# ApricityXX/PaddlePaddle

Measured on AMD Instinct MI355X. Metric: tokens/sec GPT-3-13B sharding-3 + ResNet50 img/s, at 1/2/4/8 MI355X, higher is better.
Workload: dtype bf16; 1 GPU; model=GPT-3 13B (h5120 L40 a40 ffn20480 V50304), global_batch=16, seq_len=2048, micro_batch=4, accum_steps=4, parallelism=sharding_stage3_degree1, recompute=False, fused_head_ce=False, paired_wgrad=False, optimizer=AdamW fp32-master fused HIP, amp=O2 bf16, allocator=native auto-growth best-fit

## Files before the change

### csrc/kernels/flash_attn_kernels.h

```cpp
#pragma once
#include "common.h"
#include "mfma_tile.h"

using namespace pa;

typedef __attribute__((ext_vector_type(8))) _Float16 f16x8_t;
typedef __attribute__((ext_vector_type(16))) float f32x16;

namespace pa_fa {

constexpr float kLog2e = 1.4426950408889634f;
constexpr float kLn2 = 0.6931471805599453f;

union Frag {
  bf16x8_t v;
  f16x8_t f;
  uint4 u;
  s16x4 h[2];
};

template <bool F16>
__device__ __forceinline__ f32x16 mfma32(const Frag& a, const Frag& b, f32x16 c) {
  if constexpr (F16) return __builtin_amdgcn_mfma_f32_32x32x16_f16(a.f, b.f, c, 0, 0, 0);
  else return __builtin_amdgcn_mfma_f32_32x32x16_bf16(a.v, b.v, c, 0, 0, 0);
// ... 606 lines not shown
  const int h0 = hk * G;
  const int64_t dq_row0 = varlen ? (int64_t)q_start : (int64_t)b * p.Sq;
  auto head_range = [&](int h, int& qa, int& qe) {
    qa = q_begin0;
    qe = Sq;
    if constexpr (kFm) {
      if (p.fm_stats != nullptr) {
        const int* st = p.fm_stats + (int64_t)b * p.fmst[0] + (int64_t)h * p.fmst[1] + (int64_t)(kb * (BK / 64)) * 8;
        int mx_lo0 = st[1], mn_lo1 = st[2], mx_up0 = st[5], mn_up1 = st[6];
#pragma unroll
        for (int tt = 1; tt < BK / 64; ++tt) {
          mx_lo0 = max(mx_lo0, st[tt * 8 + 1]); mn_lo1 = min(mn_lo1, st[tt * 8 + 2]);
          mx_up0 = max(mx_up0, st[tt * 8 + 5]); mn_up1 = min(mn_up1, st[tt * 8 + 6]);
        }
        if (mn_lo1 == 0x7fffffff) qe = min(qe, max(mx_lo0, 0));
        if (mx_up0 <= 0) qa = max(qa, min(mn_up1, Sq));
      }
    }
    qa = (qa / BM) * BM;
  };

  constexpr int QLOADS = BM * NCH / NT;
  u32x4 qreg[QLOADS], dreg[QLOADS];
  constexpr int mk = kMk;
  constexpr bool has_fm = kFm;
  float lse_raw = 0.f, dlt_raw = 0.f;
  uint32_t mreg[16];
  bool row_ok = false;
  bool q_ok[QLOADS];
  auto prefetch = [&](int h, int q0) {
    const uint16_t* qbase = p.q + (varlen ? (int64_t)q_start * p.qs[1] : (int64_t)b * p.qs[0]) + (int64_t)h * p.qs[2];
    const uint16_t* dobase =
        p.dout + (varlen ? (int64_t)q_start * p.dos[1] : (int64_t)b * p.dos[0]) + (int64_t)h * p.dos[2];
#pragma unroll
    for (int i = 0; i < QLOADS; ++i) {
      const int idx = tid + NT * i;
      const int row = idx / NCH, ch = idx % NCH;
      const int qx = q0 + row;
      q_ok[i] = qx < Sq;
      const int qc = q_ok[i] ? qx : Sq - 1;
      qreg[i] = gload16_async(qbase + (int64_t)qc * p.qs[1] + ch * 8);
      dreg[i] = gload16_async(dobase + (int64_t)qc * p.dos[1] + ch * 8);
    }
    const int qx = q0 + (tid & (BM - 1));
    row_ok = qx < Sq;
    const int qc = row_ok ? qx : Sq - 1;
    const int64_t lrow = (int64_t)b * p.lse_s[0] + (int64_t)h * p.lse_s[1] + q_start + qc;
    lse_raw = __uint_as_float(gload4_async(p.lse + lrow));
    dlt_raw = __uint_as_float(gload4_async(p.delta + lrow));
  };
  auto mask_load = [&](int h, int q0) {
    if constexpr (kMask) {
      constexpr int esz = kMk == kMaskBool ? 1 : (kMk == kMaskBF16 ? 2 : 4);
      const char* mb = reinterpret_cast<const char*>(p.mask) + ((int64_t)b * p.ms[0] + (int64_t)h * p.ms[1]) * esz;
      const int kc = kj < Sk ? kj : 0;
#pragma unroll
      for (int i = 0; i < 16; ++i) {
        int qr = q0 + (i & 3) + 8 * (i >> 2) + 4 * hf;
        qr = qr < Sq ? qr : 0;
        const char* ad = mb + ((int64_t)qr * p.ms[2] + kc) * esz;
        if constexpr (kMk == kMaskBool) mreg[i] = gload1_async(ad);
        else if constexpr (kMk == kMaskBF16) mreg[i] = gload2_async(ad);
        else mreg[i] = gload4_async(ad);
      }
    }
  };
  const bool has_atomics = w < NDT;
  const float inv_scale = 1.f / p.scale;

  auto dq_step = [&](const char* dsb, int h, int qb0) {
    float* dqb = p.dq_acc + dq_row0 * p.H * D + (int64_t)h * D;
    const __amdgpu_buffer_rsrc_t dq_rsrc = __builtin_amdgcn_make_buffer_rsrc(
        dqb, 0, (int)((int64_t)(Sq - 1) * p.H * D * 4 + D * 4), 0x00020000);
    for (int dt = w; dt < NDT; dt += NW) {
      f32x16 qacc = zero16();
#pragma unroll
      for (int ks = 0; ks < BK / 16; ++ks) {
        Frag a, bb;
        const int kr0 = 16 * ks + 8 * hf;
        const int ra = kr0 + qq, rb = kr0 + 4 + qq;
        a.h[0] = lds_tr(dsb + (ra * (BM * 2) + (((16 * G1 + 4 * pp) * 2) ^ (((ra >> 2) & 3) << 3))));
        a.h[1] = lds_tr(dsb + (rb * (BM * 2) + (((16 * G1 + 4 * pp) * 2) ^ (((rb >> 2) & 3) << 3))));
        const int cch = (dt * 32 + 16 * G1) / 8 + (pp >> 1);
        bb.h[0] = lds_tr(k_lds + (img_off<NCH>(kr0 + qq, cch) + 8 * (pp & 1)));
        bb.h[1] = lds_tr(k_lds + (img_off<NCH>(kr0 + 4 + qq, cch) + 8 * (pp & 1)));
        qacc = mfma32<F16>(a, bb, qacc);
      }
      const int rs = p.H * D * 4;
      const int base = qb0 * rs + (dt * 32 + r) * 4;
#pragma unroll
      for (int i = 0; i < 16; ++i) {
        const int qr = (i & 3) + 8 * (i >> 2) + 4 * hf;
        const int off = (qb0 + qr < Sq && !(p.abl & 1)) ? base + qr * rs : 0x7ffffff0;
        __builtin_amdgcn_raw_ptr_buffer_atomic_fadd_f32(qacc[i] * p.scale, dq_rsrc, off, 0, 0);
      }
    }
  };


  for (int hi = 0; hi < G; ++hi) {
    const int h = h0 + hi;
    int qa, qe;
    head_range(h, qa, qe);
    const int n_qb = qa < qe ? (qe - qa + BM - 1) / BM : 0;
    if (n_qb == 0) continue;
    FmBounds fbk{0, 0, 0, 0};
    if constexpr (kFm) {
      const int* fbp = p.fm + (int64_t)b * p.fms[0] + (int64_t)h * p.fms[1] + (int64_t)(kj < Sk ? kj : 0) * p.fm_cols;
      int v4[4];
#pragma unroll
      for (int j = 0; j < 4; ++j) v4[j] = fbp[j < p.fm_cols ? j : 0];
      fbk = fm_canon(v4, p.fm_cols, p.causal);
    }
    prefetch(h, qa);
    for (int it = 0; it < n_qb; ++it) {
      const int q0 = qa + it * BM;
      if (it == 0 || !has_atomics || ATOMICS > 63) {
        asm volatile("s_waitcnt vmcnt(0)" : "+v"(qreg[0]), "+v"(dreg[0]), "+v"(lse_raw), "+v"(dlt_raw)::"memory");
      } else {
        asm volatile("s_waitcnt vmcnt(%4)" : "+v"(qreg[0]), "+v"(dreg[0]), "+v"(lse_raw), "+v"(dlt_raw)
                     : "n"(ATOMICS > 63 ? 0 : ATOMICS) : "memory");
      }
      if constexpr (QLOADS > 1) asm volatile("" : "+v"(qreg[QLOADS - 1]), "+v"(dreg[QLOADS - 1]));
#pragma unroll
      for (int i = 0; i < QLOADS; ++i) {
        if (!q_ok[i]) {
          qreg[i] = u32x4{0u, 0u, 0u, 0u};
          dreg[i] = u32x4{0u, 0u, 0u, 0u};
        }
      }
      const float lse_r = row_ok ? -lse_raw * inv_scale : -INFINITY;
      const float dlt_r = row_ok ? -dlt_raw : 0.f;
      lds_barrier();
#pragma unroll
      for (int i = 0; i < QLOADS; ++i) {
        const int idx = tid + NT * i;
        const int row = idx / NCH, ch = idx % NCH;
        *reinterpret_cast<u32x4*>(q_lds + img_off<NCH>(row, ch)) = qreg[i];
        *reinterpret_cast<u32x4*>(do_lds + img_off<NCH>(row, ch)) = dreg[i];
      }
      if (tid < BM) {
        lse_s[tid] = lse_r;
        dlt_s[tid] = dlt_r;
      }
      lds_barrier();
      if (kMask) mask_load(h, q0);
      if (it + 1 < n_qb) prefetch(h, q0 + BM);
      if (it > 0 && !(p.abl & 2)) dq_step(ds_lds + (((it - 1) & 1) * DST_BYTES), h, q0 - BM);
      const bool dq_ran = it > 0 && has_atomics;

      f32x16 sacc, pacc;
#pragma unroll
      for (int g = 0; g < 4; ++g) {
        const float4 l4 = *reinterpret_cast<const float4*>(lse_s + 8 * g + 4 * hf);
        const float4 d4 = *reinterpret_cast<const float4*>(dlt_s + 8 * g + 4 * hf);
        sacc[4 * g + 0] = l4.x; sacc[4 * g + 1] = l4.y; sacc[4 * g + 2] = l4.z; sacc[4 * g + 3] = l4.w;
        pacc[4 * g + 0] = d4.x; pacc[4 * g + 1] = d4.y; pacc[4 * g + 2] = d4.z; pacc[4 * g + 3] = d4.w;
      }
#pragma unroll
      for (int ks = 0; ks < KS; ++ks) {
        Frag qa, da;
        qa.u = lds_b128(q_lds, img_off<NCH>(r, 2 * ks + hf));
        da.u = lds_b128(do_lds, img_off<NCH>(r, 2 * ks + hf));
        if constexpr (CACHE_KV) {
          sacc = mfma32<F16>(qa, kfr[ks], sacc);
          pacc = mfma32<F16>(da, vfr[ks], pacc);
        } else {
          Frag kk, vv;
          kk.u = lds_b128(k_lds, img_off<NCH>(w * 32 + r, 2 * ks + hf));
          vv.u = lds_b128(v_lds, img_off<NCH>(w * 32 + r, 2 * ks + hf));
          sacc = mfma32<F16>(qa, kk, sacc);
          pacc = mfma32<F16>(da, vv, pacc);
        }
      }
      if constexpr (kMask) {
        const int n_after = (it + 1 < n_qb ? 2 * QLOADS + 2 : 0) + (dq_ran ? ATOMICS : 0);
        switch (n_after) {
          case 4: asm volatile("s_waitcnt vmcnt(4)" : "+v"(mreg[0]), "+v"(mreg[15]) :: "memory"); break;
          case 6: asm volatile("s_waitcnt vmcnt(6)" : "+v"(mreg[0]), "+v"(mreg[15]) :: "memory"); break;
          case 16: asm volatile("s_waitcnt vmcnt(16)" : "+v"(mreg[0]), "+v"(mreg[15]) :: "memory"); break;
          case 18: asm volatile("s_waitcnt vmcnt(18)" : "+v"(mreg[0]), "+v"(mreg[15]) :: "memory"); break;
          case 20: asm volatile("s_waitcnt vmcnt(20)" : "+v"(mreg[0]), "+v"(mreg[15]) :: "memory"); break;
          case 22: asm volatile("s_waitcnt vmcnt(22)" : "+v"(mreg[0]), "+v"(mreg[15]) :: "memory"); break;
          case 34: asm volatile("s_waitcnt vmcnt(34)" : "+v"(mreg[0]), "+v"(mreg[15]) :: "memory"); break;
          default: asm volatile("s_waitcnt vmcnt(0)" : "+v"(mreg[0]), "+v"(mreg[15]) :: "memory"); break;
        }
#pragma unroll
        for (int i = 1; i < 15; ++i) asm volatile("" : "+v"(mreg[i]));
      }
      if (kMask && (mk == kMaskBF16 || mk == kMaskF32)) {
#pragma unroll
        for (int i = 0; i < 16; ++i) {
          const float madd = mk == kMaskBF16 ? lo_bf16(mreg[i]) : __uint_as_float(mreg[i]);
          sacc[i] += madd * inv_scale;
        }
      }
      const bool need_mask = kj >= Sk || (p.causal && kb * BK + BK - 1 > q0 + shift) || mk == kMaskBool || kFm;
      const uint32_t ka = (uint32_t)(kj >> 1);
#pragma unroll
      for (int i = 0; i < 16; ++i) {
        const int qr = (i & 3) + 8 * (i >> 2) + 4 * hf;
        float pr = __builtin_amdgcn_exp2f(sacc[i] * p.scale_log2);
        if (need_mask) {
          bool dead = kj >= Sk || (p.causal && kj > q0 + qr + shift);
          if (kMask && mk == kMaskBool) dead = dead || (mreg[i] & 0xFFu) == 0u;
          if (kFm) dead = dead || fm_masked(fbk, q0 + qr);
          if (dead) pr = 0.f;
        }
        if (kDrop) {
          const uint32_t qa = (uint32_t)(q0 + qr) ^ ((uint32_t)(b * p.H + h) * 0x9E3779B1u);
          const bool keep = drop_keep(drop_hash(p.seed0, p.seed1, qa, ka), kj, p.keep16);
          const float ndelta = dlt_s[qr];
          const float dp = pacc[i] - ndelta;
          pacc[i] = pr * ((keep ? dp * p.rkeep : 0.f) + ndelta);
          sacc[i] = keep ? pr * p.rkeep : 0.f;
        } else {
          sacc[i] = pr;
          pacc[i] = pr * pacc[i];
        }
      }
      Frag pf[2], sf[2];
#pragma unroll
      for (int s = 0; s < 2; ++s) {
        float a[8], cc[8];
#pragma unroll
        for (int j = 0; j < 8; ++j) { a[j] = sacc[8 * s + j]; cc[j] = pacc[8 * s + j]; }
        pf[s] = pack8<F16>(a);
        sf[s] = pack8<F16>(cc);
      }

#pragma unroll
      for (int dt = 0; dt < NDT; ++dt) {
        if (p.abl & 4) break;
        const int cch = (dt * 32 + 16 * G1) / 8 + (pp >> 1);
        const int cb = 8 * (pp & 1);
#pragma unroll
        for (int s = 0; s < 2; ++s) {
          const int R0 = 16 * s + 4 * hf;
          Frag a, cfr;
          a.h[0] = lds_tr(do_lds + (img_off<NCH>(R0 + qq, cch) + cb));
          a.h[1] = lds_tr(do_lds + (img_off<NCH>(R0 + 8 + qq, cch) + cb));
          dv_acc[dt] = mfma32<F16>(a, pf[s], dv_acc[dt]);
          cfr.h[0] = lds_tr(q_lds + (img_off<NCH>(R0 + qq, cch) + cb));
          cfr.h[1] = lds_tr(q_lds + (img_off<NCH>(R0 + 8 + qq, cch) + cb));
          dk_acc[dt] = mfma32<F16>(cfr, sf[s], dk_acc[dt]);
        }
      }

      {
        const int row = w * 32 + r;
        char* rowp = ds_lds + (it & 1) * DST_BYTES + row * (BM * 2);
        const int sw = ((row >> 2) & 3) << 3;
#pragma unroll
        for (int s = 0; s < 2; ++s) {
          const Frag f = sf[s];
          *reinterpret_cast<uint2*>(rowp + (((16 * s + 4 * hf) * 2) ^ sw)) = make_uint2(f.u.x, f.u.y);
          *reinterpret_cast<uint2*>(rowp + (((16 * s + 8 + 4 * hf) * 2) ^ sw)) = make_uint2(f.u.z, f.u.w);
        }
      }
    }
    lds_barrier();
    if (!(p.abl & 2)) dq_step(ds_lds + (((n_qb - 1) & 1) * DST_BYTES), h, qa + (n_qb - 1) * BM);
  }

  if (kj < Sk) {
    uint16_t* dkrow = p.dk + (varlen ? (int64_t)k_start * p.dks[1] : (int64_t)b * p.dks[0]) + (int64_t)kj * p.dks[1] +
                      (int64_t)hk * p.dks[2];
    uint16_t* dvrow = p.dv + (varlen ? (int64_t)k_start * p.dvs[1] : (int64_t)b * p.dvs[0]) + (int64_t)kj * p.dvs[1] +
                      (int64_t)hk * p.dvs[2];
#pragma unroll
    for (int dt = 0; dt < NDT; ++dt) {
#pragma unroll
      for (int g = 0; g < 4; ++g) {
        const int d0 = dt * 32 + 8 * g + 4 * hf;
        uint2 a, cc;
        a.x = pack2<F16>(dk_acc[dt][4 * g] * p.scale, dk_acc[dt][4 * g + 1] * p.scale);
        a.y = pack2<F16>(dk_acc[dt][4 * g + 2] * p.scale, dk_acc[dt][4 * g + 3] * p.scale);
        cc.x = pack2<F16>(dv_acc[dt][4 * g], dv_acc[dt][4 * g + 1]);
        cc.y = pack2<F16>(dv_acc[dt][4 * g + 2], dv_acc[dt][4 * g + 3]);
        *reinterpret_cast<uint2*>(dkrow + d0) = a;
        *reinterpret_cast<uint2*>(dvrow + d0) = cc;
      }
    }
  }
}



template <bool F16>
__device__ __forceinline__ f32x4 mfma16(const Frag& a, const Frag& b, f32x4 c) {
  if constexpr (F16) return __builtin_amdgcn_mfma_f32_16x16x32_f16(a.f, b.f, c, 0, 0, 0);
  else return __builtin_amdgcn_mfma_f32_16x16x32_bf16(a.v, b.v, c, 0, 0, 0);
}

__device__ __forceinline__ int fa_swz(int row) { return (0x78 >> (2 * ((row >> 2) & 3))) & 3; }
__device__ __forceinline__ int img_a(int row, int ch) {
  return 2048 * (row >> 3) + 512 * (ch >> 2) + 64 * (row & 7) + 16 * ((ch & 3) ^ fa_swz(row));
}

__device__ __forceinline__ int dst_off(int row, int col4) {
  return row * 64 + ((col4 ^ ((row >> 1) & 7)) << 3);
}

template <bool F16, bool DSQ>
__global__ __launch_bounds__(512, 1) void fa_bwd16_kernel(BwdArgs p) {
  constexpr int D = 128, NCH = 16, NW = 8, NT = NW * 64, BK = 128, BM = 32;
  constexpr int KT_BYTES = BK * D * 2;
  constexpr int QT_BYTES = BM * D * 2;
  constexpr int DST_BYTES = BK * BM * 2;
  __shared__ __attribute__((aligned(16))) char smem[2 * KT_BYTES + 4 * QT_BYTES + 2 * DST_BYTES + 2 * 2 * BM * 4];
  char* k_lds = smem;
  char* v_lds = smem + KT_BYTES;
  char* q_st = v_lds + KT_BYTES;
  char* do_st = q_st + 2 * QT_BYTES;
  char* ds_lds = do_st + 2 * QT_BYTES;
  char* rc_st = ds_lds + 2 * DST_BYTES;

  const int nkb0 = (p.Sk + BK - 1) / BK;
  int kb, bhk;
  block_map((int)blockIdx.x, p.B * p.Hk, nkb0, p.grp, bhk, kb);
  const int b = bhk / p.Hk, hk = bhk % p.Hk;
  const int G = p.H / p.Hk;
  int q_start = 0, k_start = 0, Sq = p.Sq, Sk = p.Sk;
  const bool varlen = p.cu_q != nullptr;
  if (varlen) {
    q_start = p.cu_q[b];
    Sq = p.cu_q[b + 1] - q_start;
    k_start = p.cu_k[b];
    Sk = p.cu_k[b + 1] - k_start;
  }
  if (kb * BK >= Sk) return;
  const int tid = threadIdx.x, w = tid >> 6, lane = tid & 63, r16 = lane & 15, kg = lane >> 4;
  const int tq = r16 >> 2, tp = r16 & 3;
  const int shift = Sk - Sq;
  const int kj = kb * BK + w * 16 + r16;

  const uint16_t* kbase = p.k + (varlen ? (int64_t)k_start * p.ks[1] : (int64_t)b * p.ks[0]) + (int64_t)hk * p.ks[2];
  const uint16_t* vbase = p.v + (varlen ? (int64_t)k_start * p.vs[1] : (int64_t)b * p.vs[0]) + (int64_t)hk * p.vs[2];
#pragma unroll
  for (int i = 0; i < BK * NCH / NT; ++i) {
    const int idx = tid + NT * i;
    const int row = idx / NCH, ch = idx % NCH;
    const int key = kb * BK + row;
    uint4 val = make_uint4(0, 0, 0, 0), vv = make_uint4(0, 0, 0, 0);
    if (key < Sk) {
      val = *reinterpret_cast<const uint4*>(kbase + (int64_t)key * p.ks[1] + ch * 8);
      vv = *reinterpret_cast<const uint4*>(vbase + (int64_t)key * p.vs[1] + ch * 8);
    }
    *reinterpret_cast<uint4*>(k_lds + img_a(row, ch)) = val;
    *reinterpret_cast<uint4*>(v_lds + img_a(row, ch)) = vv;
  }
  f32x4 dk_acc[8], dv_acc[8];
#pragma unroll
  for (int dt = 0; dt < 8; ++dt)
#pragma unroll
    for (int i = 0; i < 4; ++i) { dk_acc[dt][i] = 0.f; dv_acc[dt][i] = 0.f; }
  __syncthreads();
  Frag kfr[4], vfr[4];
#pragma unroll
  for (int ks = 0; ks < 4; ++ks) {
    kfr[ks].u = lds_b128(k_lds, img_a(w * 16 + r16, 4 * ks + kg));
    vfr[ks].u = lds_b128(v_lds, img_a(w * 16 + r16, 4 * ks + kg));
  }

  int q_begin0 = 0;
  if (p.causal) q_begin0 = max(0, kb * BK - shift);
  q_begin0 = DSQ ? (q_begin0 / 128) * 128 : (q_begin0 / BM) * BM;
  const int h0 = hk * G;
  const int64_t dq_row0 = varlen ? (int64_t)q_start : (int64_t)b * p.Sq;

  const int o_dst = 1024 * w + 16 * lane;
  const int pf_row = 8 * (o_dst >> 11) + ((o_dst & 511) >> 6);
  const int pf_ch = 4 * ((o_dst & 2047) >> 9) + (((o_dst & 63) >> 4) ^ fa_swz(pf_row));
  auto prefetch = [&](int h, int q0, int sl) {
    const uint16_t* qbase = p.q + (varlen ? (int64_t)q_start * p.qs[1] : (int64_t)b * p.qs[0]) + (int64_t)h * p.qs[2];
    const uint16_t* dobase =
        p.dout + (varlen ? (int64_t)q_start * p.dos[1] : (int64_t)b * p.dos[0]) + (int64_t)h * p.dos[2];
    const int qx = q0 + pf_row;
    const int qc = qx < Sq ? qx : Sq - 1;
    glds16(qbase + (int64_t)qc * p.qs[1] + pf_ch * 8, q_st + sl * QT_BYTES + 1024 * w);
    glds16(dobase + (int64_t)qc * p.dos[1] + pf_ch * 8, do_st + sl * QT_BYTES + 1024 * w);
    if (w == 0) {
      const int qr = q0 + (lane & 31);
      const int qrc = qr < Sq ? qr : Sq - 1;
      const int64_t lrow = (int64_t)b * p.lse_s[0] + (int64_t)h * p.lse_s[1] + q_start + qrc;
      glds4(lane < 32 ? (const void*)(p.lse + lrow) : (const void*)(p.delta + lrow), rc_st + sl * 256);
    }
  };
  const float inv_scale = 1.f / p.scale;

  auto dq_step = [&](const char* dsb, int h, int qb0) {
    float* dqb = p.dq_acc + dq_row0 * p.H * D + (int64_t)h * D;
    const __amdgpu_buffer_rsrc_t dq_rsrc = __builtin_amdgcn_make_buffer_rsrc(
        dqb, 0, (int)((int64_t)(Sq - 1) * p.H * D * 4 + D * 4), 0x00020000);
    f32x4 qacc[2];
#pragma unroll
    for (int qt = 0; qt < 2; ++qt)
#pragma unroll
      for (int i = 0; i < 4; ++i) qacc[qt][i] = 0.f;
    const int kb0 = img_a(8 * kg + tq, 2 * w + (tp >> 1)) + 8 * (tp & 1);
    const int kb4 = img_a(8 * kg + 4 + tq, 2 * w + (tp >> 1)) + 8 * (tp & 1);
    const int sb0 = dst_off(8 * kg + tq, tp), sb4 = dst_off(8 * kg + 4 + tq, tp);
#pragma unroll
    for (int ks = 0; ks < 4; ++ks) {
      Frag bb;
      bb.h[0] = lds_tr(k_lds + (kb0 + 8192 * ks));
      bb.h[1] = lds_tr(k_lds + (kb4 + 8192 * ks));
#pragma unroll
      for (int qt = 0; qt < 2; ++qt) {
        Frag a;
        a.h[0] = lds_tr(dsb + ((sb0 ^ (32 * qt)) + 2048 * ks));
        a.h[1] = lds_tr(dsb + ((sb4 ^ (32 * qt)) + 2048 * ks));
        qacc[qt] = mfma16<F16>(a, bb, qacc[qt]);
      }
      if (ks & 1) __builtin_amdgcn_sched_barrier(0);
    }
    const int rs = p.H * D * 4;
#pragma unroll
    for (int qt = 0; qt < 2; ++qt)
#pragma unroll
      for (int i = 0; i < 4; ++i) {
        const int qr = 16 * qt + 4 * kg + i;
        const int off = (qb0 + qr < Sq) ? (qb0 + qr) * rs + (16 * w + r16) * 4 : 0x7ffffff0;
        __builtin_amdgcn_raw_ptr_buffer_atomic_fadd_f32(qacc[qt][i] * p.scale, dq_rsrc, off, 0, 0);
      }
  };
  const int st_ks = w >> 1, st_qt = w & 1;
  const int st_o0 = (dst_off(8 * kg + tq, tp) ^ (32 * st_qt)) + 2048 * st_ks;
  const int st_o1 = (dst_off(8 * kg + 4 + tq, tp) ^ (32 * st_qt)) + 2048 * st_ks;
  const int64_t nkg = p.ds_rows / 32;
  auto ds_store = [&](const char* dsb, int h, int qb0) {
    Frag a;
    a.h[0] = lds_tr(dsb + st_o0);
    a.h[1] = lds_tr(dsb + st_o1);
    const u32x4 v = {a.u.x, a.u.y, a.u.z, a.u.w};
    uint16_t* dst = p.ds + (((int64_t)(b * p.H + h) * nkg + kb * 4 + st_ks) * p.ds_ld + qb0 + 16 * st_qt + r16) * 32 +
                    8 * kg;
    asm volatile("global_store_dwordx4 %0, %1, off" ::"v"(dst), "v"(v) : "memory");
  };

  for (int hi = 0; hi < G; ++hi) {
    const int h = h0 + hi;
    const int qa = q_begin0;
    const int n_qb = qa < Sq ? (Sq - qa + BM - 1) / BM : 0;
    if (n_qb == 0) continue;
    prefetch(h, qa, 0);
    for (int it = 0; it <= n_qb; ++it) {
      const int q0 = qa + it * BM;
      const bool last = it == n_qb;
      const int sl = it & 1;
      if (!last) {
        if (it >= 2) {
          if constexpr (DSQ) asm volatile("s_waitcnt vmcnt(1)" ::: "memory");
          else asm volatile("s_waitcnt vmcnt(8)" ::: "memory");
        } else {
          asm volatile("s_waitcnt vmcnt(0)" ::: "memory");
        }
      }
      lds_barrier();
      if (!last && it + 1 < n_qb) prefetch(h, q0 + BM, sl ^ 1);
      if constexpr (DSQ) {
        if (it > 0) ds_store(ds_lds + (((it - 1) & 1) * DST_BYTES), h, q0 - BM);
      } else {
        if (it > 0 && p.k16 == 1) dq_step(ds_lds + (((it - 1) & 1) * DST_BYTES), h, q0 - BM);
      }
      if (last) break;

      const char* q_lds = q_st + sl * QT_BYTES;
      const char* do_lds = do_st + sl * QT_BYTES;
      const float* lse_s = reinterpret_cast<const float*>(rc_st + sl * 256);
      const float* dlt_s = lse_s + BM;
      f32x4 sacc[2], pacc[2];
#pragma unroll
      for (int qt = 0; qt < 2; ++qt) {
        const float4 l4 = *reinterpret_cast<const float4*>(lse_s + 16 * qt + 4 * kg);
        const float4 d4 = *reinterpret_cast<const float4*>(dlt_s + 16 * qt + 4 * kg);
        const float lv[4] = {l4.x, l4.y, l4.z, l4.w}, dv4[4] = {d4.x, d4.y, d4.z, d4.w};
#pragma unroll
        for (int i = 0; i < 4; ++i) {
          const bool ok = q0 + 16 * qt + 4 * kg + i < Sq;
          sacc[qt][i] = ok ? -lv[i] * inv_scale : -INFINITY;
          pacc[qt][i] = ok ? -dv4[i] : 0.f;
        }
      }
      const int rb = img_a(r16, kg);
#pragma unroll
      for (int ks = 0; ks < 4; ++ks) {
#pragma unroll
        for (int qt = 0; qt < 2; ++qt) {
          Frag qf, df;
          qf.u = lds_b128(q_lds, rb + 4096 * qt + 512 * ks);
          df.u = lds_b128(do_lds, rb + 4096 * qt + 512 * ks);
          sacc[qt] = mfma16<F16>(qf, kfr[ks], sacc[qt]);
          pacc[qt] = mfma16<F16>(df, vfr[ks], pacc[qt]);
        }
        if (ks & 1) __builtin_amdgcn_sched_barrier(0);
      }
      const bool need_mask = kj >= Sk || (p.causal && kb * BK + BK - 1 > q0 + shift);
      float pv[8], sv[8];
#pragma unroll
      for (int qt = 0; qt < 2; ++qt)
#pragma unroll
        for (int i = 0; i < 4; ++i) {
          const int qr = 16 * qt + 4 * kg + i;
          float pr = __builtin_amdgcn_exp2f(sacc[qt][i] * p.scale_log2);
          if (need_mask && (kj >= Sk || (p.causal && kj > q0 + qr + shift))) pr = 0.f;
          pv[4 * qt + i] = pr;
          sv[4 * qt + i] = pr * pacc[qt][i];
          if (p.k16 >= 3) {
            pv[4 * qt + i] = p.k16 == 3 ? 1.f : sacc[qt][i];
            sv[4 * qt + i] = pacc[qt][i];
          }
        }
      const Frag pf = pack8<F16>(pv), sf = pack8<F16>(sv);

      const int tb0 = img_a(4 * kg + tq, tp >> 1) + 8 * (tp & 1);
      const int tb1 = img_a(4 * kg + tq, 2 + (tp >> 1)) + 8 * (tp & 1);
#pragma unroll
      for (int dt = 0; dt < 8; ++dt) {
        const int tb = ((dt & 1) ? tb1 : tb0) + 512 * (dt >> 1);
        Frag a, c;
        a.h[0] = lds_tr(do_lds + tb);
        a.h[1] = lds_tr(do_lds + (tb + 4096));
        dv_acc[dt] = mfma16<F16>(a, pf, dv_acc[dt]);
        c.h[0] = lds_tr(q_lds + tb);
        c.h[1] = lds_tr(q_lds + (tb + 4096));
        dk_acc[dt] = mfma16<F16>(c, sf, dk_acc[dt]);
        if (dt & 1) __builtin_amdgcn_sched_barrier(0);
      }
      {
        char* dsb = ds_lds + (it & 1) * DST_BYTES;
        const int row = w * 16 + r16;
        *reinterpret_cast<uint2*>(dsb + dst_off(row, kg)) = make_uint2(sf.u.x, sf.u.y);
        *reinterpret_cast<uint2*>(dsb + dst_off(row, 4 + kg)) = make_uint2(sf.u.z, sf.u.w);
      }
    }
  }

  if (kj < Sk) {
    uint16_t* dkrow = p.dk + (varlen ? (int64_t)k_start * p.dks[1] : (int64_t)b * p.dks[0]) + (int64_t)kj * p.dks[1] +
                      (int64_t)hk * p.dks[2];
    uint16_t* dvrow = p.dv + (varlen ? (int64_t)k_start * p.dvs[1] : (int64_t)b * p.dvs[0]) + (int64_t)kj * p.dvs[1] +
                      (int64_t)hk * p.dvs[2];
#pragma unroll
    for (int dt = 0; dt < 8; ++dt) {
      const int d0 = 16 * dt + 4 * kg;
      uint2 a, cc;
      a.x = pack2<F16>(dk_acc[dt][0] * p.scale, dk_acc[dt][1] * p.scale);
      a.y = pack2<F16>(dk_acc[dt][2] * p.scale, dk_acc[dt][3] * p.scale);
      cc.x = pack2<F16>(dv_acc[dt][0], dv_acc[dt][1]);
      cc.y = pack2<F16>(dv_acc[dt][2], dv_acc[dt][3]);
      *reinterpret_cast<uint2*>(dkrow + d0) = a;
      *reinterpret_cast<uint2*>(dvrow + d0) = cc;
    }
  }
}

__device__ __forceinline__ Frag dq_frag(const char* img, int rbase, int lane) {
  const int g = lane >> 4, i = lane & 15, q = i >> 2, pp = i & 3;
  const int col = rbase + pp * 4;
  const int lc = col >> 3, sub = (col & 7) * 2;
  const int k1 = g * 8 + q, k2 = k1 + 4;
  Frag f;
  f.h[0] = lds_tr(img + (k1 * 256 + ((lc ^ mn_swz(k1)) << 4) + sub));
  f.h[1] = lds_tr(img + (k2 * 256 + ((lc ^ mn_swz(k2)) << 4) + sub));
  return f;
}

__device__ __forceinline__ void dq_wait_after(int n) {
  if (n >= 2) asm volatile("s_waitcnt vmcnt(8)" ::: "memory");
  else if (n == 1) asm volatile("s_waitcnt vmcnt(4)" ::: "memory");
  else asm volatile("s_waitcnt vmcnt(0)" ::: "memory");
}

template <bool F16>
__global__ __launch_bounds__(256, 2) void fa_bwd_dq_kernel(BwdArgs p) {
  constexpr int TB = 32 * 128 * 2;
  constexpr int NS = 4;
  __shared__ __attribute__((aligned(1024))) char smem[NS * 2 * TB];
  const int nqb = (p.Sq + 127) / 128;
  int bh, rank;
  block_map((int)blockIdx.x, p.B * p.H, nqb, p.dq_grp, bh, rank);
  const int qb = p.causal ? (nqb - 1 - rank) : rank;
  const int b = bh / p.H, h = bh % p.H, hk = h / (p.H / p.Hk);
  const int q0 = qb * 128;
  const int shift = p.Sk - p.Sq;
  const int tid = threadIdx.x, w = tid >> 6, lane = tid & 63;
  const int wm = w >> 1, wn = w & 1;
  int kend = p.Sk;
  if (p.causal) kend = min(p.Sk, min(q0 + 127, p.Sq - 1) + shift + 1);
  const int nkt = kend > 0 ? (kend + 31) / 32 : 0;

  const uint16_t* ds = p.ds + ((int64_t)bh * (p.ds_rows / 32) * p.ds_ld + q0) * 32;
  const int64_t ds_grp = p.ds_ld * 32;
  const uint16_t* kb = p.k + (int64_t)b * p.ks[0] + (int64_t)hk * p.ks[2];
  int aoff[2], srow[2], scol[2];
#pragma unroll
  for (int i = 0; i < 2; ++i) {
    const int lin = (i * 4 + w) * 64 + lane;
    const int arow = lin >> 2;
    aoff[i] = arow * 32 + (((lin & 3) ^ k32_swz(arow)) * 8);
    srow[i] = lin >> 4;
    scol[i] = ((lin & 15) ^ mn_swz(srow[i])) * 8;
  }
  auto issue = [&](int t) {
    char* a_img = smem + (t % NS) * 2 * TB;
    char* b_img = a_img + TB;
#pragma unroll
    for (int i = 0; i < 2; ++i) {
      glds16(ds + t * ds_grp + aoff[i], a_img + (i * 4 + w) * 1024);
      const int key = t * 32 + srow[i];
      const int kc = key < p.Sk ? key : p.Sk - 1;
      glds16(kb + (int64_t)kc * p.ks[1] + scol[i], b_img + (i * 4 + w) * 1024);
    }
  };

  f32x4 acc[4][4];
#pragma unroll
  for (int i = 0; i < 4; ++i)
#pragma unroll
    for (int j = 0; j < 4; ++j) acc[i][j] = f32x4{0.f, 0.f, 0.f, 0.f};

  for (int t = 0; t < min(nkt, NS - 1); ++t) issue(t);
  for (int t = 0; t < nkt; ++t) {
    dq_wait_after(min(nkt - 1 - t, NS - 2));
    lds_barrier();
    if (t + NS - 1 < nkt) issue(t + NS - 1);
    const char* a_img = smem + (t % NS) * 2 * TB;
    const char* b_img = a_img + TB;
    Frag af[4], bf[4];
#pragma unroll
    for (int i = 0; i < 4; ++i) {
      const int row = wm * 64 + i * 16 + (lane & 15);
      af[i].u = lds_b128(a_img, row * 64 + (((lane >> 4) ^ k32_swz(row)) << 4));
    }
#pragma unroll
    for (int j = 0; j < 4; ++j) bf[j] = dq_frag(b_img, wn * 64 + j * 16, lane);
#pragma unroll
    for (int i = 0; i < 4; ++i)
#pragma unroll
      for (int j = 0; j < 4; ++j) acc[i][j] = mfma16<F16>(bf[j], af[i], acc[i][j]);
  }
  uint16_t* dqb = p.dq + (int64_t)b * p.dqs[0] + (int64_t)h * p.dqs[2];
#pragma unroll
  for (int i = 0; i < 4; ++i) {
    const int q = q0 + wm * 64 + i * 16 + (lane & 15);
    if (q >= p.Sq) continue;
#pragma unroll
    for (int j = 0; j < 4; ++j) {
      const int d = wn * 64 + j * 16 + 4 * (lane >> 4);
      uint2 o;
      o.x = pack2<F16>(acc[i][j][0] * p.scale, acc[i][j][1] * p.scale);
      o.y = pack2<F16>(acc[i][j][2] * p.scale, acc[i][j][3] * p.scale);
      *reinterpret_cast<uint2*>(dqb + (int64_t)q * p.dqs[1] + d) = o;
    }
  }
}

template <int D, bool F16, int MW>
void fa_fwd_feat(const FwdArgs& a, int feat, dim3 grid, hipStream_t st) {
  switch (feat) {
    case 0: hipLaunchKernelGGL((fa_fwd_kernel<D, F16, MW, 0>), grid, dim3(256), 0, st, a); break;
    case 1: hipLaunchKernelGGL((fa_fwd_kernel<D, F16, MW, 1>), grid, dim3(256), 0, st, a); break;
    case 2: hipLaunchKernelGGL((fa_fwd_kernel<D, F16, MW, 2>), grid, dim3(256), 0, st, a); break;
    case 4: hipLaunchKernelGGL((fa_fwd_kernel<D, F16, MW, 4>), grid, dim3(256), 0, st, a); break;
    case 5: hipLaunchKernelGGL((fa_fwd_kernel<D, F16, MW, 5>), grid, dim3(256), 0, st, a); break;
    case 6: hipLaunchKernelGGL((fa_fwd_kernel<D, F16, MW, 6>), grid, dim3(256), 0, st, a); break;
    case 8: hipLaunchKernelGGL((fa_fwd_kernel<D, F16, MW, 8>), grid, dim3(256), 0, st, a); break;
    case 12: hipLaunchKernelGGL((fa_fwd_kernel<D, F16, MW, 12>), grid, dim3(256), 0, st, a); break;
    case 16: hipLaunchKernelGGL((fa_fwd_kernel<D, F16, MW, 16>), grid, dim3(256), 0, st, a); break;
    case 20: hipLaunchKernelGGL((fa_fwd_kernel<D, F16, MW, 20>), grid, dim3(256), 0, st, a); break;
    default: break;
  }
}

template <bool F16>
void fa_fwd_dispatch(const FwdArgs& a, int D, int feat, dim3 grid, hipStream_t st) {
  if (D == 128) fa_fwd_feat<128, F16, 2>(a, feat, grid, st);
  else if (D == 64) fa_fwd_feat<64, F16, 2>(a, feat, grid, st);
  else fa_fwd_feat<256, F16, 1>(a, feat, grid, st);
}

template <int D, bool F16, int NW, bool CK>
void fa_bwd_feat(const BwdArgs& a, int feat, dim3 grid, hipStream_t st) {
  switch (feat) {
    case 0: hipLaunchKernelGGL((fa_bwd_kernel<D, F16, NW, CK, 0>), grid, dim3(NW * 64), 0, st, a); break;
    case 1: hipLaunchKernelGGL((fa_bwd_kernel<D, F16, NW, CK, 1>), grid, dim3(NW * 64), 0, st, a); break;
    case 2: hipLaunchKernelGGL((fa_bwd_kernel<D, F16, NW, CK, 2>), grid, dim3(NW * 64), 0, st, a); break;
    case 4: hipLaunchKernelGGL((fa_bwd_kernel<D, F16, NW, CK, 4>), grid, dim3(NW * 64), 0, st, a); break;
    case 5: hipLaunchKernelGGL((fa_bwd_kernel<D, F16, NW, CK, 5>), grid, dim3(NW * 64), 0, st, a); break;
    case 6: hipLaunchKernelGGL((fa_bwd_kernel<D, F16, NW, CK, 6>), grid, dim3(NW * 64), 0, st, a); break;
    case 8: hipLaunchKernelGGL((fa_bwd_kernel<D, F16, NW, CK, 8>), grid, dim3(NW * 64), 0, st, a); break;
    case 12: hipLaunchKernelGGL((fa_bwd_kernel<D, F16, NW, CK, 12>), grid, dim3(NW * 64), 0, st, a); break;
    case 16: hipLaunchKernelGGL((fa_bwd_kernel<D, F16, NW, CK, 16>), grid, dim3(NW * 64), 0, st, a); break;
    case 20: hipLaunchKernelGGL((fa_bwd_kernel<D, F16, NW, CK, 20>), grid, dim3(NW * 64), 0, st, a); break;
    default: break;
  }
}

template <bool F16>
void fa_bwd_dispatch(const BwdArgs& a, int D, int feat, dim3 grid, hipStream_t st) {
  if (D == 128 && feat == 0 && a.ds != nullptr) {
    hipLaunchKernelGGL((fa_bwd16_kernel<F16, true>), grid, dim3(512), 0, st, a);
    const int nqb = (a.Sq + 127) / 128;
    hipLaunchKernelGGL((fa_bwd_dq_kernel<F16>), dim3((unsigned)(a.B * a.H * nqb)), dim3(256), 0, st, a);
    return;
  }
  if (D == 128 && feat == 0 && a.k16 && a.abl == 0) {
    hipLaunchKernelGGL((fa_bwd16_kernel<F16, false>), grid, dim3(512), 0, st, a);
    return;
  }
  if (D == 128) fa_bwd_feat<128, F16, 4, true>(a, feat, grid, st);
  else if (D == 64) fa_bwd_feat<64, F16, 4, true>(a, feat, grid, st);
  else fa_bwd_feat<256, F16, 2, false>(a, feat, grid, st);
}

template <bool F16>
void fa_bwd_aux(int which, const BwdArgs& a, const uint16_t* o, const uint16_t* dout, float* delta, const int64_t* os,
                const int64_t* dos, const float* dq_acc, uint16_t* dq, const int64_t* dqs, int DB, int DS, int H, int D,
                hipStream_t st) {
  if (which == 0) {
    const int64_t threads = (int64_t)DB * DS * H * (D / 8);
    hipLaunchKernelGGL(fa_bwd_delta<F16>, dim3((unsigned)cdiv(threads, 256)), dim3(256), 0, st, o, dout, delta, os[0],
                       os[1], os[2], dos[0], dos[1], dos[2], DB, DS, H, D, a.lse_s[0], a.lse_s[1]);
  } else {
    const int64_t nvec = (int64_t)DB * DS * H * D / 8;
    int64_t g = cdiv(nvec, 256);
    if (g > 4096) g = 4096;
    hipLaunchKernelGGL(fa_bwd_dq_convert<F16>, dim3((unsigned)g), dim3(256), 0, st, dq_acc, dq, dqs[0], dqs[1], dqs[2],
                       DB, DS, H, D);
  }
}

}
using namespace pa_fa;

void pa_fa_fwd_f16(const FwdArgs& a, int D, int feat, dim3 grid, hipStream_t st);
void pa_fa_bwd_f16(const BwdArgs& a, int D, int feat, dim3 grid, hipStream_t st);
void pa_fa_bwd_aux_f16(int which, const BwdArgs& a, const uint16_t* o, const uint16_t* dout, float* delta,
                       const int64_t* os, const int64_t* dos, const float* dq_acc, uint16_t* dq, const int64_t* dqs,
                       int DB, int DS, int H, int D, hipStream_t st);
```

### csrc/kernels/mfma_tile.h

```cpp
#pragma once
#include "common.h"

namespace pa {

typedef __attribute__((ext_vector_type(8))) __bf16 bf16x8_t;
typedef __attribute__((ext_vector_type(4))) float f32x4;
typedef __attribute__((ext_vector_type(4))) short s16x4;
typedef __attribute__((ext_vector_type(4))) int i32x4;
typedef __attribute__((ext_vector_type(4))) unsigned int u32x4;

union Frag8 {
  bf16x8_t v;
  uint4 u;
  u32x4 w;
  s16x4 h[2];
};

__device__ __forceinline__ void glds16(const void* g, const char* lds_wave_base) {
  const uint32_t m0 = __builtin_amdgcn_readfirstlane((uint32_t)reinterpret_cast<uintptr_t>(lds_wave_base));
  asm volatile("s_mov_b32 m0, %1\n\ts_nop 0\n\tglobal_load_lds_dwordx4 %0, off" ::"v"(g), "s"(m0) : "memory", "m0");
}
__device__ __forceinline__ void glds4(const void* g, const char* lds_wave_base) {
  const uint32_t m0 = __builtin_amdgcn_readfirstlane((uint32_t)reinterpret_cast<uintptr_t>(lds_wave_base));
  asm volatile("s_mov_b32 m0, %1\n\ts_nop 0\n\tglobal_load_lds_dword %0, off" ::"v"(g), "s"(m0) : "memory", "m0");
}

__device__ __forceinline__ s16x4 lds_tr(const char* p) {
  return __builtin_amdgcn_ds_read_tr16_b64_v4i16(
      (__attribute__((address_space(3))) s16x4*)(reinterpret_cast<uintptr_t>(p)));
}

__device__ __forceinline__ void bar() {
  asm volatile("" ::: "memory");
  __builtin_amdgcn_s_barrier();
  asm volatile("" ::: "memory");
  __builtin_amdgcn_sched_barrier(0);
}

__device__ __forceinline__ void vm_wait(int n) {
  switch (n) {
    case 0: asm volatile("s_waitcnt vmcnt(0)" ::: "memory"); break;
    case 2: asm volatile("s_waitcnt vmcnt(2)" ::: "memory"); break;
    case 4: asm volatile("s_waitcnt vmcnt(4)" ::: "memory"); break;
    case 6: asm volatile("s_waitcnt vmcnt(6)" ::: "memory"); break;
    case 8: asm volatile("s_waitcnt vmcnt(8)" ::: "memory"); break;
    case 10: asm volatile("s_waitcnt vmcnt(10)" ::: "memory"); break;
    default: asm volatile("s_waitcnt vmcnt(0)" ::: "memory"); break;
  }
}

constexpr __host__ __device__ __forceinline__ int k_swz(int row) { return (row >> 1) & 7; }
constexpr __host__ __device__ __forceinline__ int k32_swz(int row) { return ((row >> 3) & 1) << 1; }
constexpr __host__ __device__ __forceinline__ int mn_swz(int k) { return ((k & 3) | (((k >> 3) & 1) << 2)) << 1; }
template <int R>
constexpr __host__ __device__ __forceinline__ int mn_swz_r(int k) { return mn_swz(k) & (R / 8 - 1); }

template <int R>
constexpr bool mn_swz_ok() {
  for (int k = 0; k < 64; ++k) {
    const int s = mn_swz_r<R>(k);
    if (s % 2 != 0 || (R >= 128 && s != mn_swz(k))) return false;
    for (int c = 0; c < R / 8; ++c)
      if ((c ^ s) >= R / 8) return false;
  }
  return true;
}
static_assert(mn_swz_ok<64>() && mn_swz_ok<128>() && mn_swz_ok<256>(), "MN-major swizzle");

template <int R, bool KMAJ, int NW = 8, class T>
__device__ __forceinline__ void stage(const T* __restrict__ g, int64_t ld, int r0, int rmax, int k0, char* img,
                                      int wave, int lane) {
  constexpr int E = 16 / sizeof(T);
  constexpr int NQ = R / (8 * NW);
  static_assert(KMAJ || sizeof(T) == 2, "MN-major images hold 16-bit elements");
#pragma unroll
  for (int i = 0; i < NQ; ++i) {
    const int q = i * NW + wave;
    if constexpr (KMAJ) {
      const int row = q * 8 + (lane >> 3);
      const int lc = (lane & 7) ^ k_swz(row);
      int gr = r0 + row;
      gr = gr < rmax ? gr : rmax - 1;
      glds16(g + (int64_t)gr * ld + k0 + lc * E, img + q * 1024);
    } else {
      constexpr int CPR = R / 8;
      const int lin = q * 64 + lane;
      const int row = lin / CPR;
      const int lc = (lin % CPR) ^ mn_swz_r<R>(row);
      int gc = r0 + lc * 8;
      gc = gc < rmax ? gc : rmax - 8;
      glds16(g + (int64_t)(k0 + row) * ld + gc, img + q * 1024);
    }
  }
}

template <int R, bool KMAJ>
__device__ __forceinline__ bf16x8_t frag(const char* img, int rbase, int s, int lane) {
  Frag8 f;
  if constexpr (KMAJ) {
    const int row = rbase + (lane & 15);
    const int c = s * 4 + (lane >> 4);
    f.u = *reinterpret_cast<const uint4*>(img + row * 128 + ((c ^ k_swz(row)) << 4));
  } else {
    const int g = lane >> 4, i = lane & 15, q = i >> 2, pp = i & 3;
    const int col = rbase + pp * 4;
    const int lc = col >> 3, sub = (col & 7) * 2;
    const int k1 = s * 32 + g * 8 + q, k2 = k1 + 4;
    f.h[0] = lds_tr(img + k1 * (R * 2) + ((lc ^ mn_swz_r<R>(k1)) << 4) + sub);
    f.h[1] = lds_tr(img + k2 * (R * 2) + ((lc ^ mn_swz_r<R>(k2)) << 4) + sub);
  }
  return f.v;
}

__device__ __forceinline__ int xcd_remap(int bid, int nwg) {
  const int xcd = bid & 7, q = nwg >> 3, r = nwg & 7;
  return (xcd < r ? xcd * (q + 1) : r * (q + 1) + (xcd - r) * q) + (bid >> 3);
}

__device__ __forceinline__ void tile_coords(int pid, int tiles_m, int tiles_n, int* tm, int* tn) {
  constexpr int GM = 8;
  const int per_group = GM * tiles_n;
  const int first_m = (pid / per_group) * GM;
  const int gsz = min(tiles_m - first_m, GM);
  *tm = first_m + (pid % per_group) % gsz;
  *tn = (pid % per_group) / gsz;
}

template <int V>
struct IntC {
  static constexpr int value = V;
};

}
```

Before: 13810 tokens/s.

## Software-pipeline LDS reads against MFMAs in flash-attention backward k16 kernel

Restructures the inner loop of the 16x16 flash-attention backward kernel. Q/dO fragment reads and transposed reads are now issued a few steps ahead of the MFMAs that use them, using rotating register slots and sched_group_barrier interleaving in place of full sched_barriers. Adds a wave-uniform fast path that skips per-element masking when the tile is full. Moves the k16>=3 debug overrides into a separate template instantiation so they leave the hot kernel. This aims to hide LDS latency and remove masking ALU work, at the cost of higher register pressure from the extra fragment buffers.

```diff
diff --git a/csrc/kernels/flash_attn_kernels.h b/csrc/kernels/flash_attn_kernels.h
--- a/csrc/kernels/flash_attn_kernels.h
+++ b/csrc/kernels/flash_attn_kernels.h
@@ -932,12 +932,15 @@
   return row * 64 + ((col4 ^ ((row >> 1) & 7)) << 3);
 }
 
-template <bool F16, bool DSQ>
+template <bool F16, bool DSQ, bool DBG = false>
 __global__ __launch_bounds__(512, 1) void fa_bwd16_kernel(BwdArgs p) {
+  static_assert(!(DSQ && DBG), "the debug levels run on the atomics route");
   constexpr int D = 128, NCH = 16, NW = 8, NT = NW * 64, BK = 128, BM = 32;
   constexpr int KT_BYTES = BK * D * 2;
   constexpr int QT_BYTES = BM * D * 2;
   constexpr int DST_BYTES = BK * BM * 2;
+  constexpr int DO_OFF = 2 * QT_BYTES;
+  constexpr int SA = DSQ ? 3 : 1, TD = DSQ ? 2 : 1;
   __shared__ __attribute__((aligned(16))) char smem[2 * KT_BYTES + 4 * QT_BYTES + 2 * DST_BYTES + 2 * 2 * BM * 4];
   char* k_lds = smem;
   char* v_lds = smem + KT_BYTES;
@@ -964,6 +967,7 @@
   const int tq = r16 >> 2, tp = r16 & 3;
   const int shift = Sk - Sq;
   const int kj = kb * BK + w * 16 + r16;
+  const int wk0 = kb * BK + __builtin_amdgcn_readfirstlane(w) * 16;
 
   const uint16_t* kbase = p.k + (varlen ? (int64_t)k_start * p.ks[1] : (int64_t)b * p.ks[0]) + (int64_t)hk * p.ks[2];
   const uint16_t* vbase = p.v + (varlen ? (int64_t)k_start * p.vs[1] : (int64_t)b * p.vs[0]) + (int64_t)hk * p.vs[2];
@@ -1017,7 +1021,7 @@
       glds4(lane < 32 ? (const void*)(p.lse + lrow) : (const void*)(p.delta + lrow), rc_st + sl * 256);
     }
   };
-  const float inv_scale = 1.f / p.scale;
+  const float inv_scale = 1.f / p.scale, scale_log2 = p.scale_log2;
 
   auto dq_step = [&](const char* dsb, int h, int qb0) {
     float* dqb = p.dq_acc + dq_row0 * p.H * D + (int64_t)h * D;
@@ -1097,66 +1101,115 @@
       if (last) break;
 
       const char* q_lds = q_st + sl * QT_BYTES;
-      const char* do_lds = do_st + sl * QT_BYTES;
       const float* lse_s = reinterpret_cast<const float*>(rc_st + sl * 256);
       const float* dlt_s = lse_s + BM;
+      const bool need_mask = wk0 + 15 >= Sk || (p.causal && wk0 + 15 > q0 + shift);
+      const bool full = q0 + BM <= Sq && !need_mask;
       f32x4 sacc[2], pacc[2];
-#pragma unroll
-      for (int qt = 0; qt < 2; ++qt) {
-        const float4 l4 = *reinterpret_cast<const float4*>(lse_s + 16 * qt + 4 * kg);
-        const float4 d4 = *reinterpret_cast<const float4*>(dlt_s + 16 * qt + 4 * kg);
-        const float lv[4] = {l4.x, l4.y, l4.z, l4.w}, dv4[4] = {d4.x, d4.y, d4.z, d4.w};
-#pragma unroll
-        for (int i = 0; i < 4; ++i) {
-          const bool ok = q0 + 16 * qt + 4 * kg + i < Sq;
-          sacc[qt][i] = ok ? -lv[i] * inv_scale : -INFINITY;
-          pacc[qt][i] = ok ? -dv4[i] : 0.f;
-        }
-      }
-      const int rb = img_a(r16, kg);
-#pragma unroll
-      for (int ks = 0; ks < 4; ++ks) {
+      if (full) {
 #pragma unroll
         for (int qt = 0; qt < 2; ++qt) {
-          Frag qf, df;
-          qf.u = lds_b128(q_lds, rb + 4096 * qt + 512 * ks);
-          df.u = lds_b128(do_lds, rb + 4096 * qt + 512 * ks);
-          sacc[qt] = mfma16<F16>(qf, kfr[ks], sacc[qt]);
-          pacc[qt] = mfma16<F16>(df, vfr[ks], pacc[qt]);
-        }
-        if (ks & 1) __builtin_amdgcn_sched_barrier(0);
-      }
-      const bool need_mask = kj >= Sk || (p.causal && kb * BK + BK - 1 > q0 + shift);
+          const float4 l4 = *reinterpret_cast<const float4*>(lse_s + 16 * qt + 4 * kg);
+          const float4 d4 = *reinterpret_cast<const float4*>(dlt_s + 16 * qt + 4 * kg);
+          sacc[qt] = f32x4{-l4.x * inv_scale, -l4.y * inv_scale, -l4.z * inv_scale, -l4.w * inv_scale};
+          pacc[qt] = f32x4{-d4.x, -d4.y, -d4.z, -d4.w};
+        }
+      } else {
+        asm volatile("");
+#pragma unroll
+        for (int qt = 0; qt < 2; ++qt) {
+          const float4 l4 = *reinterpret_cast<const float4*>(lse_s + 16 * qt + 4 * kg);
+          const float4 d4 = *reinterpret_cast<const float4*>(dlt_s + 16 * qt + 4 * kg);
+          const float lv[4] = {l4.x, l4.y, l4.z, l4.w}, dv4[4] = {d4.x, d4.y, d4.z, d4.w};
+#pragma unroll
+          for (int i = 0; i < 4; ++i) {
+            const bool ok = q0 + 16 * qt + 4 * kg + i < Sq;
+            sacc[qt][i] = ok ? -lv[i] * inv_scale : -INFINITY;
+            pacc[qt][i] = ok ? -dv4[i] : 0.f;
+          }
+        }
+      }
+      const uint32_t rq = lds_base(q_lds + img_a(r16, kg));
+      const uint32_t tq0 = lds_base(q_lds + img_a(4 * kg + tq, tp >> 1) + 8 * (tp & 1));
+      const uint32_t tq1 = lds_base(q_lds + img_a(4 * kg + tq, 2 + (tp >> 1)) + 8 * (tp & 1));
+      Frag qf[SA + 1], df[SA + 1];
+      auto read_sp = [&](int slot, int u) {
+        qf[slot].v = lds_b128_at(rq, 4096 * (u & 1) + 512 * (u >> 1));
+        df[slot].v = lds_b128_at(rq, DO_OFF + 4096 * (u & 1) + 512 * (u >> 1));
+      };
+      Frag ta[TD + 1], tc[TD + 1];
+      auto read_t = [&](int slot, int dt) {
+        const uint32_t tb = (dt & 1) ? tq1 : tq0;
+        const int o = 512 * (dt >> 1);
+        ta[slot].h[0] = lds_tr_at(tb, DO_OFF + o);
+        ta[slot].h[1] = lds_tr_at(tb, DO_OFF + o + 4096);
+        tc[slot].h[0] = lds_tr_at(tb, o);
+        tc[slot].h[1] = lds_tr_at(tb, o + 4096);
+      };
+#pragma unroll
+      for (int u = 0; u < SA; ++u) read_sp(u, u);
+      __builtin_amdgcn_sched_group_barrier(0x100, 2 * SA, 0);
+#pragma unroll
+      for (int u = 0; u < 8; ++u) {
+        if (u + SA < 8) {
+          read_sp((u + SA) % (SA + 1), u + SA);
+          __builtin_amdgcn_sched_group_barrier(0x100, 2, 0);
+        } else if (u + SA == 8) {
+#pragma unroll
+          for (int dt = 0; dt < TD; ++dt) read_t(dt, dt);
+          __builtin_amdgcn_sched_group_barrier(0x100, 4 * TD, 0);
+        }
+        sacc[u & 1] = mfma16<F16>(qf[u % (SA + 1)], kfr[u >> 1], sacc[u & 1]);
+        pacc[u & 1] = mfma16<F16>(df[u % (SA + 1)], vfr[u >> 1], pacc[u & 1]);
+        __builtin_amdgcn_sched_group_barrier(0x008, 2, 0);
+      }
       float pv[8], sv[8];
-#pragma unroll
-      for (int qt = 0; qt < 2; ++qt)
-#pragma unroll
-        for (int i = 0; i < 4; ++i) {
-          const int qr = 16 * qt + 4 * kg + i;
-          float pr = __builtin_amdgcn_exp2f(sacc[qt][i] * p.scale_log2);
-          if (need_mask && (kj >= Sk || (p.causal && kj > q0 + qr + shift))) pr = 0.f;
-          pv[4 * qt + i] = pr;
-          sv[4 * qt + i] = pr * pacc[qt][i];
-          if (p.k16 >= 3) {
-            pv[4 * qt + i] = p.k16 == 3 ? 1.f : sacc[qt][i];
-            sv[4 * qt + i] = pacc[qt][i];
+      int full_v = full;
+      asm volatile("" : "+v"(full_v));
+      if (__builtin_amdgcn_readfirstlane(full_v)) {
+#pragma unroll
+        for (int qt = 0; qt < 2; ++qt)
+#pragma unroll
+          for (int i = 0; i < 4; ++i) {
+            const float pr = __builtin_amdgcn_exp2f(sacc[qt][i] * scale_log2);
+            pv[4 * qt + i] = pr;
+            sv[4 * qt + i] = pr * pacc[qt][i];
           }
-        }
+      } else {
+        const int klim = p.causal ? q0 + shift : 0x3fffffff;
+        const int kq = kj >= Sk ? 0x7fffff00 : kj - 4 * kg;
+#pragma unroll
+        for (int qt = 0; qt < 2; ++qt)
+#pragma unroll
+          for (int i = 0; i < 4; ++i) {
+            const float e = __builtin_amdgcn_exp2f(sacc[qt][i] * scale_log2);
+            const float pr = kq - (16 * qt + i) > klim ? 0.f : e;
+            pv[4 * qt + i] = pr;
+            sv[4 * qt + i] = pr * pacc[qt][i];
+          }
+      }
+      if constexpr (DBG) {
+        if (p.k16 >= 3) {
+#pragma unroll
+          for (int qt = 0; qt < 2; ++qt)
+#pragma unroll
+            for (int i = 0; i < 4; ++i) {
+              pv[4 * qt + i] = p.k16 == 3 ? 1.f : sacc[qt][i];
+              sv[4 * qt + i] = pacc[qt][i];
+            }
+        }
+      }
       const Frag pf = pack8<F16>(pv), sf = pack8<F16>(sv);
 
-      const int tb0 = img_a(4 * kg + tq, tp >> 1) + 8 * (tp & 1);
-      const int tb1 = img_a(4 * kg + tq, 2 + (tp >> 1)) + 8 * (tp & 1);
 #pragma unroll
       for (int dt = 0; dt < 8; ++dt) {
-        const int tb = ((dt & 1) ? tb1 : tb0) + 512 * (dt >> 1);
-        Frag a, c;
-        a.h[0] = lds_tr(do_lds + tb);
-        a.h[1] = lds_tr(do_lds + (tb + 4096));
-        dv_acc[dt] = mfma16<F16>(a, pf, dv_acc[dt]);
-        c.h[0] = lds_tr(q_lds + tb);
-        c.h[1] = lds_tr(q_lds + (tb + 4096));
-        dk_acc[dt] = mfma16<F16>(c, sf, dk_acc[dt]);
-        if (dt & 1) __builtin_amdgcn_sched_barrier(0);
+        if (dt + TD < 8) {
+          read_t((dt + TD) % (TD + 1), dt + TD);
+          __builtin_amdgcn_sched_group_barrier(0x100, 4, 0);
+        }
+        dv_acc[dt] = mfma16<F16>(ta[dt % (TD + 1)], pf, dv_acc[dt]);
+        dk_acc[dt] = mfma16<F16>(tc[dt % (TD + 1)], sf, dk_acc[dt]);
+        __builtin_amdgcn_sched_group_barrier(0x008, 2, 0);
       }
       {
         char* dsb = ds_lds + (it & 1) * DST_BYTES;
@@ -1337,7 +1390,8 @@
     return;
   }
   if (D == 128 && feat == 0 && a.k16 && a.abl == 0) {
-    hipLaunchKernelGGL((fa_bwd16_kernel<F16, false>), grid, dim3(512), 0, st, a);
+    if (a.k16 >= 3) hipLaunchKernelGGL((fa_bwd16_kernel<F16, false, true>), grid, dim3(512), 0, st, a);
+    else hipLaunchKernelGGL((fa_bwd16_kernel<F16, false>), grid, dim3(512), 0, st, a);
     return;
   }
   if (D == 128) fa_bwd_feat<128, F16, 4, true>(a, feat, grid, st);
diff --git a/csrc/kernels/mfma_tile.h b/csrc/kernels/mfma_tile.h
--- a/csrc/kernels/mfma_tile.h
+++ b/csrc/kernels/mfma_tile.h
@@ -28,6 +28,19 @@
 __device__ __forceinline__ s16x4 lds_tr(const char* p) {
   return __builtin_amdgcn_ds_read_tr16_b64_v4i16(
       (__attribute__((address_space(3))) s16x4*)(reinterpret_cast<uintptr_t>(p)));
+}
+
+__device__ __forceinline__ uint32_t lds_base(const char* p) {
+  uint32_t a = (uint32_t)reinterpret_cast<uintptr_t>(p);
+  asm("" : "+v"(a));
+  return a;
+}
+__device__ __forceinline__ bf16x8_t lds_b128_at(uint32_t base, int off) {
+  return *(__attribute__((address_space(3))) const bf16x8_t*)(uintptr_t)(base + (uint32_t)off);
+}
+__device__ __forceinline__ s16x4 lds_tr_at(uint32_t base, int off) {
+  return __builtin_amdgcn_ds_read_tr16_b64_v4i16(
+      (__attribute__((address_space(3))) s16x4*)(uintptr_t)(base + (uint32_t)off));
 }
 
 __device__ __forceinline__ void bar() {
```

Measured after the change: 13940 tokens/s, median of 6. About the same (+0.9%).
